# lhaippp/DMHomo

Hardware: AMD Instinct MI355X
Metric: sampled images/sec (128x128, s_step=32) (higher is better)
Workload: dtype f32; 1 GPU; DGM CFG-Unet dim=64 128x128 bs=25/GPU s_step=32 cond_scale=3 (BASELINE configs[1]); global_batch=25, cfg_mode=streams, hip_graph=True, weights=seeded random init

## Files before the change

dmhomo_amd/csrc/conv_f16x3.hip:

```cpp
#include <stdlib.h>

#include "common.h"

#include "conv_args.h"
#include "weight_image.h"

typedef _Float16 half8 __attribute__((ext_vector_type(8)));
typedef _Float16 half4 __attribute__((ext_vector_type(4)));
typedef float float4v __attribute__((ext_vector_type(4)));

namespace {

constexpr int KC = 32;
constexpr int PITCH = 160;
constexpr int STEP_U4 = 4 * 64;

template <int KH, int KW, int S, int UPS, int TH, int TW, int WM, int WN>
struct F16Cfg {
  static_assert(WM * WN == 4, "four waves per workgroup");
  static constexpr bool SUB = UPS == 3;
  static_assert(SUB || TH * TW == WM * 64, "64 pixels per wave");
  static_assert(!SUB || (KH == 2 && KW == 2 && S == 1 && TH == 4 && TW == 16 && WM == 4 && WN == 1), "sub-pixel geometry");
  static constexpr int IN_H = SUB ? TH + 2 : (TH - 1) * S + KH;
  static constexpr int IN_W = SUB ? TW + 2 : (TW - 1) * S + KW;
  static constexpr int IN_PIX = IN_H * IN_W;
  static constexpr int QS = UPS == 4 ? 2 : 3, NQ = 1 << QS;
  static constexpr int NLOAD = (IN_PIX * NQ + 255) / 256;
  static constexpr int PAD = UPS == 2 ? 0 : ((S == 1) ? (KH / 2) : (KH == 4 ? 1 : 0));
  static constexpr int ROWP = IN_W * PITCH;
  static constexpr int IN_BYTES = IN_H * ROWP;
  static constexpr int EPI_BYTES = 4 * 32 * EpilogueRows::EP * 4;
  static constexpr int TILE_BYTES = IN_BYTES > EPI_BYTES ? IN_BYTES : EPI_BYTES;
  static constexpr int LDS_BYTES = TILE_BYTES + 16;
};

__device__ __forceinline__ unsigned absbits(float x) { return __float_as_uint(x) & 0x7fffffffu; }

__device__ __forceinline__ int64_t f16x3_frag_floats_dev(int Cout, int C0, int C1, int T) {
  return (int64_t)((Cout + 63) / 64) * ((C0 + KC - 1) / KC + (C1 + KC - 1) / KC) * T * 2 * STEP_U4 * 4;
}

}

template <int KH, int KW, int S, int UPS, int TH, int TW, int WM, int WN>
__global__ __launch_bounds__(256, 2) void conv_f16x3_kernel(ConvArgs p) {
  using Cfg = F16Cfg<KH, KW, S, UPS, TH, TW, WM, WN>;
  constexpr bool PK = UPS == 4;
  constexpr int IN_W = Cfg::IN_W, IN_PIX = Cfg::IN_PIX, NLOAD = Cfg::NLOAD, NTAPS = PK ? (KH * KW + 1) / 2 : KH * KW,
                ROWP = Cfg::ROWP;

  extern __shared__ __attribute__((aligned(16))) float lds[];
  unsigned char* in_tile = reinterpret_cast<unsigned char*>(lds);
  unsigned* mxslot = reinterpret_cast<unsigned*>(in_tile + Cfg::TILE_BYTES);

  const int tid = threadIdx.x;
  const int lane = tid & 63;
  const int wave = tid >> 6;
  const int wave_u = __builtin_amdgcn_readfirstlane(wave);
  const int kg = lane >> 4;
  const int l15 = lane & 15;
  const int wm = wave / WN, wn = wave % WN;

  int t = blockIdx.x, by = blockIdx.y, nb = gridDim.x;
  if (p.rows) {
    nb = p.tilesX * p.tilesY * p.rows[0];
    const int lin = t + by * (int)gridDim.x;
    if (lin >= nb * (int)gridDim.y) return;
    t = lin % nb;
    by = lin / nb;
  }
  if (p.xcd) {
    const int total = nb * gridDim.y, lin = t + by * nb;
    const int q = total >> 3, r = total & 7, xcd = lin & 7, local = lin >> 3;
    const int nl = xcd * q + min(xcd, r) + local;
    if (p.xcd == 2) {
      by = nl % (int)gridDim.y;
      t = nl / (int)gridDim.y;
    } else {
      t = nl % nb;
      by = nl / nb;
    }
  }
  const int tx = t % p.tilesX;
  t /= p.tilesX;
  const int ty = t % p.tilesY;
  const int b = dmh_rows_phys(p.rows, t / p.tilesY);
  const int nt = UPS == 3 ? wm * (int)gridDim.y + by : by * WN + wn;
  const int n0 = UPS == 3 ? by * 64 : nt * 64;

  const int oy0 = ty * TH, ox0 = tx * TW;
  const int iy0 = oy0 * S - Cfg::PAD, ix0 = ox0 * S - Cfg::PAD;
  const int Hlim = UPS == 1 ? p.Hin * 2 : (UPS == 2 ? p.Hin / 2 + 1 : p.Hin);
  const int Wlim = UPS == 1 ? p.Win * 2 : (UPS == 2 ? p.Win / 2 + 1 : p.Win);

  if (tid < 2) mxslot[tid] = 0u;
#ifdef DMH_STAMPS
  unsigned long long tk[8] = {0, 0, 0, 0, 0, 0, 0, 0};
  unsigned long long t_prev, t_now;
#define STAMP(i)                                                                 \
  __builtin_amdgcn_sched_barrier(0);                                             \
  asm volatile("s_memtime %0\n\ts_waitcnt lgkmcnt(0)" : "=s"(t_now)::"memory"); \
  __builtin_amdgcn_sched_barrier(0);                                             \
  tk[i] += t_now - t_prev;                                                       \
  t_prev = t_now;
  asm volatile("s_memtime %0\n\ts_waitcnt lgkmcnt(0)" : "=s"(t_prev)::"memory");
  const unsigned long long t_begin = t_prev;
  const unsigned long long rt_begin = __builtin_amdgcn_s_memrealtime();
#else
#define STAMP(i)
#endif

  static_assert(TW == 16, "a 16-row MFMA block is one tile row");
  int arow[4];
#pragma unroll
  for (int mb = 0; mb < 4; ++mb)
    arow[mb] = UPS == 3 ? (mb + (wm >> 1)) * ROWP + (l15 + (wm & 1)) * PITCH + kg * 16
                        : ((wm * 4 + mb) * S) * ROWP + (l15 * S) * PITCH + (PK ? (kg & 1) : kg) * 16;

  float4v acc[4][4];
#pragma unroll
  for (int mb = 0; mb < 4; ++mb)
#pragma unroll
    for (int nb = 0; nb < 4; ++nb) acc[mb][nb] = float4v{0.f, 0.f, 0.f, 0.f};

  const int nchunks = p.nch0 + p.nch1;
  const int nsteps = nchunks * NTAPS * 2;
  const uint4* wbase = reinterpret_cast<const uint4*>(p.wpack) + (size_t)__builtin_amdgcn_readfirstlane(nt) * nsteps * STEP_U4;

  constexpr bool ROWREUSE = KH == 3 && KW == 3 && S == 1 && UPS != 3 && UPS != 2;
  constexpr int NSTEP = NTAPS * 2;
  constexpr int NB = (NSTEP % 3 == 0 && WN != 1) ? 3 : 2;
  uint4 bq[NB][4];
  auto tap_of = [](int pos) constexpr { return ROWREUSE ? (pos % 3) * 3 + pos / 3 : pos; };
  auto load_b = [&](int buf, int ch_, int st_) {
    if (st_ >= NSTEP) {
      st_ -= NSTEP;
      ch_ += 1;
    }
    if (ch_ >= nchunks) ch_ = nchunks - 1;
    const uint4* src = wbase + ((size_t)(ch_ * NTAPS + tap_of(st_ >> 1)) * 2 + (st_ & 1)) * STEP_U4;
#pragma unroll
    for (int i = 0; i < 4; ++i) bq[buf][i] = src[i * 64 + lane];
  };
#pragma unroll
  for (int i = 0; i < NB - 1; ++i) load_b(i, 0, i);

  constexpr int QS = Cfg::QS, NQ = Cfg::NQ;
  const int c4 = tid & (NQ - 1);
  float4 v[NLOAD];
  constexpr bool PACKPW = KH == 3 && KW == 3 && S == 1 && UPS == 0 && WN == 1;
  int poff[NLOAD], wroff[PACKPW ? 1 : NLOAD];
  const int y0c = min(max(iy0, 0), Hlim - 1), x0c = min(max(ix0, 0), Wlim - 1);
  const int pbase = PACKPW ? (b * p.Hin + y0c) * p.Win + x0c : 0;
  unsigned inside = 0;
#pragma unroll
  for (int i = 0; i < NLOAD; ++i) {
    const int pix = (tid + i * 256) >> QS;
    const int pixc = pix < IN_PIX ? pix : IN_PIX - 1;
    const int wro = (pixc / IN_W) * ROWP + (pixc % IN_W) * PITCH + c4 * 8;
    if (!PACKPW) wroff[i] = wro;
    const int yy = iy0 + pixc / IN_W, xx = ix0 + pixc % IN_W;
    const bool ok = pix < IN_PIX && yy >= 0 && yy < Hlim && xx >= 0 && xx < Wlim;
    const int yc = min(max(yy, 0), Hlim - 1), xc = min(max(xx, 0), Wlim - 1);
    const int sy = UPS == 1 ? (yc >> 1) : yc, sx = UPS == 1 ? (xc >> 1) : xc;
    poff[i] = UPS == 2 ? ((yc << 16) | xc) : (b * p.Hin + sy) * p.Win + sx;
    if (PACKPW) poff[i] = (int)((unsigned)wro | ((unsigned)((yc - y0c) * p.Win + (xc - x0c)) << 16));
    inside |= (ok ? 1u : 0u) << i;
  }
  unsigned inside_ch = inside;
  const float* ld_src = p.src0;
  int ld_C = p.C0, ld_c = 0, ld_py = 0, ld_px = 0;
  auto issue_prep = [&](int ch) {
    const bool s1 = ch >= p.nch0;
    ld_src = s1 ? p.src1 : p.src0;
    ld_C = s1 ? p.C1 : p.C0;
    if (UPS == 2) {
      const int nchc = p.C0 / KC, par = ch / nchc;
      ld_py = par >> 1;
      ld_px = par & 1;
      ld_c = (ch - par * nchc) * KC + c4 * 4;
      inside_ch = 0u;
    } else {
      const int c = (s1 ? ch - p.nch0 : ch) * KC + c4 * 4;
      ld_c = c < ld_C ? c : 0;
    }
  };
  auto issue_one = [&](int i) {
    const float* a;
    if (UPS == 2) {
      const int ry = 2 * (poff[i] >> 16) - 1 + ld_py, rx = 2 * (poff[i] & 0xffff) - 1 + ld_px;
      const bool ok = ((inside >> i) & 1u) && ry >= 0 && ry < p.Hin && rx >= 0 && rx < p.Win;
      const int yc = min(max(ry, 0), p.Hin - 1), xc = min(max(rx, 0), p.Win - 1);
      a = ld_src + ((size_t)(b * p.Hin + yc) * p.Win + xc) * ld_C + ld_c;
      inside_ch |= (ok ? 1u : 0u) << i;
    } else {
      if (PACKPW) a = ld_src + (size_t)pbase * ld_C + (int)(((unsigned)poff[i] >> 16) * (unsigned)ld_C + (unsigned)ld_c);
      else a = ld_src + (size_t)poff[i] * ld_C + ld_c;
    }
#ifdef DMH_STAMPS
    a = (p.ablate & 32) ? ld_src + ld_c : a;
#endif
    v[i] = ld4(a);
  };
  issue_prep(0);
#pragma unroll
  for (int i = 0; i < NLOAD; ++i) issue_one(i);
  __syncthreads();
#ifdef DMH_STAMPS
  if (p.ablate & 128) {
    const float* gs = p.src0 + (size_t)b * p.Hin * p.Win * p.C0;
    double q1 = 0.0, q2 = 0.0;
#pragma unroll
    for (int j = 0; j < 4; ++j) {
      const float2 t2 = *reinterpret_cast<const float2*>(gs + (size_t)(((tid & 31) + 32 * j) * 8 + (tid >> 5)) * 2);
      q1 += (double)t2.x;
      q2 += (double)t2.y;
    }
    for (int off = 16; off; off >>= 1) {
      q1 += __shfl_xor(q1, off);
      q2 += __shfl_xor(q2, off);
    }
    const double nn = (double)p.Hin * p.Win * (p.C0 / 8);
    const double mean = q1 / nn;
    double var = q2 / nn - mean * mean;
    var = var < 0.0 ? 0.0 : var;
    const float rstd = (float)(1.0 / sqrt(var + 1e-5)), meanf = (float)mean;
    float* tab = reinterpret_cast<float*>(in_tile);
    float* gtab = tab + 2 * 768;
    if ((tid & 31) == 0) {
      gtab[(tid >> 5) * 2 + 0] = meanf;
      gtab[(tid >> 5) * 2 + 1] = rstd;
    }
    __syncthreads();
    const float* cf = p.in_coef ? p.in_coef + (size_t)b * 2 * p.C0 : p.bias;
    for (int c = tid; c < p.C0 && c < 768; c += 256) {
      const int g8 = c / max(p.C0 / 8, 1);
      const float ga = cf ? cf[c % 64] : 1.f, be = cf ? cf[(c + 32) % 64] : 0.f;
      const float aa = gtab[g8 * 2 + 1] * ga;
      tab[c * 2 + 0] = aa;
      tab[c * 2 + 1] = be - gtab[g8 * 2 + 0] * aa;
    }
    __syncthreads();
    const float probe = tab[(tid & 63) * 2] + tab[(tid & 63) * 2 + 1];
    asm volatile("" ::"v"(probe));
    __syncthreads();
  }
#endif

  int e_run = 16;
  bool stat = p.in_bound != nullptr;
  int e_fix = 16;
  if (stat) {
    float m = 0.f;
    for (int i = 0; i < p.in_bound_n; ++i) {
      const float v = p.in_bound[b * p.in_bound_n + i];
      m = (v < INFINITY) ? fmaxf(m, v) : INFINITY;
    }
    const unsigned mb = __builtin_amdgcn_readfirstlane(__float_as_uint(m));
    stat = mb < 0x7f000000u;
    e_fix = min(max((int)(mb >> 23) + 1, 16), 254);
  }
  for (int ch = 0; ch < nchunks; ++ch) {
    const bool s1c = ch >= p.nch0;
    const bool pro = (p.in_coef != nullptr) && !s1c;
    float4 ca = make_float4(1.f, 1.f, 1.f, 1.f), cb = make_float4(0.f, 0.f, 0.f, 0.f);
    if (pro) {
      const int cq = ch * KC + c4 * 4;
      const int ccq = cq < p.C0 ? cq : 0;
      ca = ld4(p.in_coef + (size_t)(b * 2 + 0) * p.C0 + ccq);
      cb = ld4(p.in_coef + (size_t)(b * 2 + 1) * p.C0 + ccq);
    }
    const bool cvalid = UPS == 2 || (s1c ? ch - p.nch0 : ch) * KC + c4 * 4 < (s1c ? p.C1 : p.C0);
    const unsigned msk = cvalid ? inside_ch : 0u;
    if (pro) {
#pragma unroll
      for (int i = 0; i < NLOAD; ++i) {
        if ((i + 1) * 256 > IN_PIX * NQ && ((wave_u * 64 + i * 256) >> QS) >= IN_PIX) continue;
        v[i].x = silu_fast(fmaf(ca.x, v[i].x, cb.x));
        v[i].y = silu_fast(fmaf(ca.y, v[i].y, cb.y));
        v[i].z = silu_fast(fmaf(ca.z, v[i].z, cb.z));
        v[i].w = silu_fast(fmaf(ca.w, v[i].w, cb.w));
      }
    }
    if (!stat) {
      float mxf = 0.f;
#pragma unroll
      for (int i = 0; i < NLOAD; ++i) {
        if (pro && (i + 1) * 256 > IN_PIX * NQ && ((wave_u * 64 + i * 256) >> QS) >= IN_PIX) continue;
        mxf = fmaxf(fmaxf(mxf, fmaxf(fabsf(v[i].x), fabsf(v[i].y))), fmaxf(fabsf(v[i].z), fabsf(v[i].w)));
      }
      unsigned mx = __float_as_uint(mxf);
      mx = wave_max_u32(mx);
      if (lane == 0) atomicMax(&mxslot[ch & 1], mx);
    }
    STAMP(0)
    __syncthreads();
    STAMP(1)
    const int e_old = e_run;
    int e_ch = e_fix;
    if (!stat) {
      const unsigned bmx = mxslot[ch & 1];
      if (tid == 0) mxslot[(ch + 1) & 1] = 0u;
      e_ch = min(max((int)(__builtin_amdgcn_readfirstlane(bmx) >> 23), 16), 254);
    }
    e_run = max(e_run, e_ch);
    const float sc = __uint_as_float((unsigned)(268 - e_run) << 23);
    if (e_run != e_old && ch > 0) {
      const int fe = 127 + e_old - e_run;
      const float f = fe > 0 ? __uint_as_float((unsigned)fe << 23) : 0.f;
#pragma unroll
      for (int mb = 0; mb < 4; ++mb)
#pragma unroll
        for (int nb = 0; nb < 4; ++nb) acc[mb][nb] *= f;
    }
    const bool more = ch + 1 < nchunks;
    if (more) issue_prep(ch + 1);
#ifdef DMH_STAMPS
    if (p.ablate & 1) {
#pragma unroll
      for (int i = 0; i < NLOAD; ++i)
        if (more) issue_one(i);
    } else
#endif
#pragma unroll
    for (int i = 0; i < NLOAD; ++i) {
      if ((i + 1) * 256 <= IN_PIX * NQ || ((tid + i * 256) >> QS) < IN_PIX) {
        const float si = ((msk >> i) & 1u) ? sc : 0.f;
        uint2 h1, h2;
        dmh_split2(v[i].x, v[i].y, si, h1.x, h2.x);
        dmh_split2(v[i].z, v[i].w, si, h1.y, h2.y);
        int slot = PACKPW ? poff[i] : wroff[i];
        if (PACKPW) asm volatile("v_and_b32 %0, 0xffff, %0" : "+v"(slot));
        unsigned char* dst = in_tile + slot;
        *reinterpret_cast<uint2*>(dst) = h1;
        *reinterpret_cast<uint2*>(dst + 64) = h2;
      }
      if (more) issue_one(i);
    }
    STAMP(2)
    __syncthreads();
    STAMP(3)
    __builtin_amdgcn_sched_barrier(0);

    half8 a[4][2];
    half8 ar[ROWREUSE ? 5 : 1][2];
    auto read_a = [&](int tap) {
      const unsigned char* at = in_tile + (tap / KW) * ROWP + (tap % KW) * PITCH;
      if constexpr (PK) {
        const int t0 = 2 * tap, t1 = 2 * tap + 1 < KH * KW ? 2 * tap + 1 : 2 * tap;
        const int o0 = (t0 / KW) * ROWP + (t0 % KW) * PITCH, o1 = (t1 / KW) * ROWP + (t1 % KW) * PITCH;
        at = in_tile + ((kg >> 1) ? o1 : o0);
      }
#pragma unroll
      for (int mb = 0; mb < 4; ++mb)
#pragma unroll
        for (int pl = 0; pl < 2; ++pl) a[mb][pl] = *reinterpret_cast<const half8*>(at + arow[mb] + pl * 64);
    };
    auto read_rows = [&](int kx, int r0, int r1) {
      const unsigned char* at = in_tile + kx * PITCH;
#pragma unroll
      for (int r = r0; r < r1; ++r)
#pragma unroll
        for (int pl = 0; pl < 2; ++pl)
          ar[ROWREUSE ? r % 5 : 0][pl] = *reinterpret_cast<const half8*>(at + arow[0] + r * ROWP + pl * 64);
    };
#ifdef DMH_STAMPS
    if (!(p.ablate & 2))
#endif
    {
#pragma unroll
      for (int st = 0; st < NSTEP; ++st) {
#ifdef DMH_STAMPS
        if (!(p.ablate & 8))
#endif
        load_b((st + NB - 1) % NB, ch, st + NB - 1);
        __builtin_amdgcn_sched_barrier(0);
        const int pos = st >> 1;
#ifdef DMH_STAMPS
        if (!(p.ablate & 16) || st == 0)
#endif
        {
          if (ROWREUSE) {
            if ((st & 1) == 0) read_rows(pos / 3, pos % 3 == 0 ? 0 : 3 + pos % 3, 4 + pos % 3);
          } else if ((st & 1) == 0) {
            read_a(pos);
          }
        }
        auto afrag = [&](int mb, int pl) -> half8 {
          if constexpr (ROWREUSE) return ar[(mb + pos % 3) % 5][pl];
          else return a[mb][pl];
        };
#define DMH_A(mb, pl) afrag(mb, pl)
#pragma unroll
        for (int mb = 0; mb < 4; ++mb)
#pragma unroll
          for (int nb = 0; nb < 2; ++nb) {
            float4v& c = acc[mb][(st & 1) * 2 + nb];
            const half8 g1 = __builtin_bit_cast(half8, bq[st % NB][nb * 2]), g2 = __builtin_bit_cast(half8, bq[st % NB][nb * 2 + 1]);
            const half8 h1 = DMH_A(mb, 0), h2 = DMH_A(mb, 1);
            asm("v_mfma_f32_16x16x32_f16 %0, %1, %4, %0\n\t"
                "v_mfma_f32_16x16x32_f16 %0, %2, %3, %0\n\t"
                "v_mfma_f32_16x16x32_f16 %0, %1, %3, %0"
                : "+v"(c) : "v"(g1), "v"(g2), "v"(h1), "v"(h2));
          }
#undef DMH_A
      }
    }
#pragma unroll
    for (int mb = 0; mb < 4; mb += 2)
      asm volatile("s_nop 15" : "+v"(acc[mb][0]), "+v"(acc[mb][1]), "+v"(acc[mb][2]), "+v"(acc[mb][3]), "+v"(acc[mb + 1][0]),
                   "+v"(acc[mb + 1][1]), "+v"(acc[mb + 1][2]), "+v"(acc[mb + 1][3]));
    __builtin_amdgcn_sched_barrier(0);
    STAMP(4)
  }

#ifdef DMH_STAMPS
  if (!(p.ablate & 4))
#endif
  {
    constexpr int EP = EpilogueRows::EP;
    const float inv_s = __uint_as_float((unsigned)(e_run - 14) << 23);
    float* wl = lds + wave * (32 * EP);
    EpilogueRows er(p, b, n0);
    if (UPS == 3 && p.oscale) er.osc = ld4(p.oscale + nt * 64 + er.c4 * 4);
    er.osc.x *= inv_s;
    er.osc.y *= inv_s;
    er.osc.z *= inv_s;
    er.osc.w *= inv_s;
    __syncthreads();
#pragma unroll
    for (int hb = 0; hb < 2; ++hb) {
#pragma unroll
      for (int m2 = 0; m2 < 2; ++m2)
#pragma unroll
        for (int nb = 0; nb < 4; ++nb)
          *reinterpret_cast<float4v*>(wl + (m2 * 16 + l15) * EP + nb * 16 + kg * 4) = acc[hb * 2 + m2][nb];
      __builtin_amdgcn_fence(__ATOMIC_RELEASE, "wavefront");
      __builtin_amdgcn_wave_barrier();
      __builtin_amdgcn_fence(__ATOMIC_ACQUIRE, "wavefront");
      if (UPS == 3) er.template store_rows<TW>(p, wl, hb * 32, oy0, ox0, 2, wm >> 1, wm & 1);
      else er.template store_rows<TW, (KH == 1 && KW == 1 && WN == 1 && UPS == 0)>(p, wl, wm * 64 + hb * 32, oy0, ox0);
    }
#ifdef DMH_STAMPS
    STAMP(5)
    if (p.stats && lane == 0 && by == 0) {
      const int stiles = ((p.Hout + 7) / 8) * p.tilesX;
      unsigned long long* d = reinterpret_cast<unsigned long long*>(
                                  p.stats + ((size_t)(b * stiles + (ty * (TH / 8)) * p.tilesX + tx) * p.Cout) * 2) + wave * 8;
      for (int i = 0; i < 6; ++i) d[i] = tk[i];
      d[6] = t_now - t_begin;
      d[7] = __builtin_amdgcn_s_memrealtime() - rt_begin;
    }
#else
    er.template write_stats_grid<WM, WN, TH>(p, lds, ty, tx, by);
#endif
  }
}
#undef STAMP

__global__ __launch_bounds__(64) void f16x3_wscale_kernel(const float* __restrict__ w, float* __restrict__ oscale,
                                                           int Cout, int K) {
  const int o = blockIdx.x;
  float m = 0.f;
  if (o < Cout)
    for (int i = threadIdx.x; i < K; i += 64) m = fmaxf(m, fabsf(w[(size_t)o * K + i]));
  const float s = f16x3_row_scale(m);
  if (threadIdx.x == 0) oscale[o] = s;
}

__global__ void pack_f16x3_weight_kernel(const float* __restrict__ w, const float* __restrict__ oscale,
                                         _Float16* __restrict__ wp, int Cout, int C0, int NTAPS, int nch, int64_t total,
                                         int s2d) {
  const int64_t idx = (int64_t)blockIdx.x * blockDim.x + threadIdx.x;
  if (idx >= total) return;
  const F16x3Slot s = f16x3_slot(idx, NTAPS, nch);
  float ws = 0.f;
  if (s2d) {
    const int nchc = C0 / KC, par = s.ch / nchc;
    const int cr = (s.ch - par * nchc) * KC + s.k;
    const int ky = 2 * (s.tap >> 1) + (par >> 1), kx = 2 * (s.tap & 1) + (par & 1);
    if (s.o < Cout) ws = w[((size_t)s.o * C0 + cr) * 16 + ky * 4 + kx] / oscale[s.o];
  } else {
    const int tt = 2 * s.tap + (s.k >> 4), cc = s.k & 15;
    if (s.o < Cout && cc < C0 && tt < 49) ws = w[((size_t)s.o * C0 + cc) * 49 + tt] / oscale[s.o];
  }
  wp[idx] = f16x3_piece(ws, s.plane);
}

static int64_t f16x3_frag_floats(int Cout, int C0, int C1, int KH, int KW);
#define PM_MAX 32
struct PmTable {
  const float* src[PM_MAX];
  float* ws[PM_MAX];
  float* wpack[PM_MAX];
  int Cout[PM_MAX], C0[PM_MAX], C1[PM_MAX], T[PM_MAX], tr[PM_MAX];
  int blk0[PM_MAX + 1];
  int count;
};
__device__ __forceinline__ int pm_find(const PmTable& t, int blk) {
  int lo = 0, hi = t.count;
  while (hi - lo > 1) {
    const int mid = (lo + hi) >> 1;
    if (t.blk0[mid] <= blk) lo = mid; else hi = mid;
  }
  return lo;
}
__device__ __forceinline__ float pm_elem(const float* w, int o, int c, int tap, int Cout, int Cin, int T, int tr) {
  return tr ? w[((size_t)c * Cout + o) * T + (T - 1 - tap)] : w[((size_t)o * Cin + c) * T + tap];
}
__global__ __launch_bounds__(256) void pm_ws_kernel(PmTable t, float eps) {
  const int ti = pm_find(t, blockIdx.x), o = blockIdx.x - t.blk0[ti];
  const int K = (t.tr[ti] ? t.Cout[ti] : t.C0[ti] + t.C1[ti]) * t.T[ti];
  ws_standardize_row(t.src[ti] + (size_t)o * K, t.ws[ti] + (size_t)o * K, K, eps);
}
__global__ __launch_bounds__(64) void pm_wscale_kernel(PmTable t) {
  const int ti = pm_find(t, blockIdx.x), o = blockIdx.x - t.blk0[ti];
  const int Cout = t.Cout[ti], Cin = t.C0[ti] + t.C1[ti], T = t.T[ti], tr = t.tr[ti], K = Cin * T;
  const float* w = t.ws[ti] ? t.ws[ti] : t.src[ti];
  float m = 0.f;
  if (o < Cout)
    for (int i = threadIdx.x; i < K; i += 64) m = fmaxf(m, fabsf(pm_elem(w, o, i / T, i % T, Cout, Cin, T, tr)));
  const float sc = f16x3_row_scale(m);
  if (threadIdx.x == 0) t.wpack[ti][f16x3_frag_floats_dev(Cout, t.C0[ti], t.C1[ti], T) + o] = sc;
}
__global__ __launch_bounds__(256) void pm_pack_kernel(PmTable t) {
  const int ti = pm_find(t, blockIdx.x);
  const int Cout = t.Cout[ti], C0 = t.C0[ti], C1 = t.C1[ti], T = t.T[ti], tr = t.tr[ti];
  const int nch0 = (C0 + KC - 1) / KC, nch1 = (C1 + KC - 1) / KC;
  const int64_t frag = f16x3_frag_floats_dev(Cout, C0, C1, T);
  const int64_t total = frag * 2;
  const float* w = t.ws[ti] ? t.ws[ti] : t.src[ti];
  const float* oscale = t.wpack[ti] + frag;
  _Float16* wp = reinterpret_cast<_Float16*>(t.wpack[ti]);
  const int64_t base = (int64_t)(blockIdx.x - t.blk0[ti]) * 2048;
  for (int64_t idx = base + threadIdx.x; idx < min(base + 2048, total); idx += 256) {
    const F16x3Slot s = f16x3_slot(idx, T, nch0 + nch1);
    const bool src1 = s.ch >= nch0;
    const int c = (s.ch - (src1 ? nch0 : 0)) * KC + s.k;
    float ws = 0.f;
    if (c < (src1 ? C1 : C0) && s.o < Cout)
      ws = pm_elem(w, s.o, c + (src1 ? C0 : 0), s.tap, Cout, C0 + C1, T, tr) / oscale[s.o];
    wp[idx] = f16x3_piece(ws, s.plane);
  }
}

int dmh_f16x3_pack_multi(const DmhPackJob* jobs, int njobs, float eps, hipStream_t st) {
  for (int phase = 0; phase < 3; ++phase) {
    for (int i0 = 0; i0 < njobs;) {
      PmTable t;
      int k = 0, blocks = 0;
      for (; k < PM_MAX && i0 < njobs; ++i0) {
        const DmhPackJob& j = jobs[i0];
        if (phase == 0 && !j.ws) continue;
        const int T = j.KH * j.KH;
        t.src[k] = j.src;
        t.ws[k] = j.ws;
        t.wpack[k] = j.wpack;
        t.Cout[k] = j.Cout;
        t.C0[k] = j.C0;
        t.C1[k] = j.C1;
        t.T[k] = T;
        t.tr[k] = j.transposed;
        t.blk0[k] = blocks;
        if (phase == 0) blocks += j.transposed ? j.C0 + j.C1 : j.Cout;
        else if (phase == 1) blocks += cdiv(j.Cout, 64) * 64;
        else blocks += (int)cdiv64(f16x3_frag_floats(j.Cout, j.C0, j.C1, j.KH, j.KH) * 2, 2048);
        ++k;
      }
      if (k == 0) continue;
      t.blk0[k] = blocks;
      t.count = k;
      if (phase == 0) hipLaunchKernelGGL(pm_ws_kernel, dim3(blocks), dim3(256), 0, st, t, eps);
      else if (phase == 1) hipLaunchKernelGGL(pm_wscale_kernel, dim3(blocks), dim3(64), 0, st, t);
      else hipLaunchKernelGGL(pm_pack_kernel, dim3(blocks), dim3(256), 0, st, t);
      DMH_CHECK_LAUNCH("dmh_pack_conv_weights_multi");
    }
  }
  return DMH_OK;
}

static bool f16x3_pk(int C0, int C1, int KH) { return KH == 7 && C1 == 0 && C0 <= 16; }

static int64_t f16x3_frag_floats(int Cout, int C0, int C1, int KH, int KW) {
  if (KH == 4) return (int64_t)cdiv(Cout, 64) * (4 * C0 / KC) * 4 * 2 * STEP_U4 * 4;
  if (f16x3_pk(C0, C1, KH)) return (int64_t)cdiv(Cout, 64) * 25 * 2 * STEP_U4 * 4;
  return (int64_t)cdiv(Cout, 64) * (cdiv(C0, KC) + cdiv(C1, KC)) * KH * KW * 2 * STEP_U4 * 4;
}

int64_t dmh_f16x3_pack_floats(int Cout, int C0, int C1, int KH, int KW) {
  return f16x3_frag_floats(Cout, C0, C1, KH, KW) + (int64_t)cdiv(Cout, 64) * 64;
}

int dmh_f16x3_pack(const float* w, float* wpack, int Cout, int C0, int C1, int KH, int KW, hipStream_t st) {
  const bool s2d = KH == 4;
  if (!s2d && !f16x3_pk(C0, C1, KH)) {
    const DmhPackJob job = {w, nullptr, wpack, Cout, C0, C1, KH, 0};
    return dmh_f16x3_pack_multi(&job, 1, 0.f, st);
  }
  const int64_t frag = f16x3_frag_floats(Cout, C0, C1, KH, KW);
  float* oscale = wpack + frag;
  hipLaunchKernelGGL(f16x3_wscale_kernel, dim3(cdiv(Cout, 64) * 64), dim3(64), 0, st, w, oscale, Cout, C0 * KH * KW);
  const int64_t total = frag * 2;
  hipLaunchKernelGGL(pack_f16x3_weight_kernel, dim3((unsigned)cdiv64(total, 256)), dim3(256), 0, st, w, oscale,
                     reinterpret_cast<_Float16*>(wpack), Cout, C0, s2d ? 4 : 25, s2d ? 4 * C0 / KC : 1, total, s2d ? 1 : 0);
  DMH_CHECK_LAUNCH("dmh_pack_conv_weight(f16x3)");
  return DMH_OK;
}

template <int KH, int KW, int S, int UPS, int TH, int TW, int WM, int WN>
static int launch_f16x3(const DmhConv* d, int Hout, int Wout, hipStream_t st) {
  using Cfg = F16Cfg<KH, KW, S, UPS, TH, TW, WM, WN>;
  ConvArgs a = fill_conv_args(d, Hout, Wout, KC, TH, TW);
  if (UPS == 2) a.nch0 = 4 * a.C0 / KC;
  a.oscale = d->wpack + f16x3_frag_floats(d->Cout, a.C0, a.C1, UPS == 2 ? 4 : KH, UPS == 2 ? 4 : KW);
#ifdef DMH_STAMPS
  if (const char* e = getenv("DMH_WINO_ABLATE")) a.ablate = atoi(e);
#endif
  auto kern = conv_f16x3_kernel<KH, KW, S, UPS, TH, TW, WM, WN>;
  DMH_RAISE_LDS_ONCE(kern, Cfg::LDS_BYTES, "dmh_conv2d(f16x3)");
  static const int xcd_deep = [] {
    const char* e = getenv("DMH_CONV_XCD_DEEP");
    return e ? atoi(e) : 32;
  }();
  if (xcd_deep > 0 && Hout <= xcd_deep && cdiv(a.Cout, 64 * WN) > 1) a.xcd = 2;
  dim3 grid(a.tilesX * a.tilesY * a.B, cdiv(a.Cout, 64 * WN));
  hipLaunchKernelGGL(kern, grid, dim3(256), Cfg::LDS_BYTES, st, a);
  DMH_CHECK_LAUNCH("dmh_conv2d(f16x3)");
  return DMH_OK;
}

__global__ void subpixel_weight_kernel(const float* __restrict__ w, float* __restrict__ wv, int Cout, int Cin) {
  const int64_t idx = (int64_t)blockIdx.x * blockDim.x + threadIdx.x;
  const int64_t total = (int64_t)4 * Cout * Cin * 4;
  if (idx >= total) return;
  const int tb = idx & 1, ta = (idx >> 1) & 1;
  int64_t r = idx >> 2;
  const int c = r % Cin;
  r /= Cin;
  const int o = r % Cout, par = r / Cout;
  const int dy = par >> 1, dx = par & 1;
  const int ky0 = dy == 0 ? (ta == 0 ? 0 : 1) : (ta == 0 ? 0 : 2), ky1 = dy == 0 ? (ta == 0 ? 0 : 2) : (ta == 0 ? 1 : 2);
  const int kx0 = dx == 0 ? (tb == 0 ? 0 : 1) : (tb == 0 ? 0 : 2), kx1 = dx == 0 ? (tb == 0 ? 0 : 2) : (tb == 0 ? 1 : 2);
  const float* wk = w + ((size_t)o * Cin + c) * 9;
  float s = 0.f;
  for (int ky = ky0; ky <= ky1; ++ky)
    for (int kx = kx0; kx <= kx1; ++kx) s += wk[ky * 3 + kx];
  wv[idx] = s;
}

int64_t dmh_f16x3_up2_pack_floats(int Cout, int C0) {
  return dmh_f16x3_pack_floats(4 * Cout, C0, 0, 2, 2) + (int64_t)16 * Cout * C0;
}

int dmh_f16x3_up2_pack(const float* w, float* wpack, int Cout, int C0, hipStream_t st) {
  float* wv = wpack + dmh_f16x3_pack_floats(4 * Cout, C0, 0, 2, 2);
  const int64_t total = (int64_t)16 * Cout * C0;
  hipLaunchKernelGGL(subpixel_weight_kernel, dim3((unsigned)cdiv64(total, 256)), dim3(256), 0, st, w, wv, Cout, C0);
  return dmh_f16x3_pack(wv, wpack, 4 * Cout, C0, 0, 2, 2, st);
}

int dmh_f16x3_launch_up2(const DmhConv* d, int Hout, int Wout, hipStream_t st) {
  using Cfg = F16Cfg<2, 2, 1, 3, 4, 16, 4, 1>;
  ConvArgs a = fill_conv_args(d, Hout, Wout, KC, 4, 16);
  a.tilesX = cdiv(d->Win, 16);
  a.tilesY = cdiv(d->Hin, 4);
  a.oscale = d->wpack + f16x3_frag_floats(4 * d->Cout, a.C0, 0, 2, 2);
  auto kern = conv_f16x3_kernel<2, 2, 1, 3, 4, 16, 4, 1>;
  DMH_RAISE_LDS_ONCE(kern, Cfg::LDS_BYTES, "dmh_conv2d(f16x3 sub-pixel)");
  dim3 grid(a.tilesX * a.tilesY * a.B, cdiv(a.Cout, 64));
  hipLaunchKernelGGL(kern, grid, dim3(256), Cfg::LDS_BYTES, st, a);
  DMH_CHECK_LAUNCH("dmh_conv2d(f16x3 sub-pixel)");
  return DMH_OK;
}

int dmh_f16x3_launch(const DmhConv* d, int Hout, int Wout, hipStream_t st) {
  const bool wide = d->Cout % 128 == 0;
  if (d->KH == 4) {
    return wide ? launch_f16x3<2, 2, 1, 2, 8, 16, 2, 2>(d, Hout, Wout, st)
                : launch_f16x3<2, 2, 1, 2, 16, 16, 4, 1>(d, Hout, Wout, st);
  }
  if (d->KH == 7) {
    if (f16x3_pk(d->C0, d->src1 ? d->C1 : 0, 7)) return launch_f16x3<7, 7, 1, 4, 16, 16, 4, 1>(d, Hout, Wout, st);
    return launch_f16x3<7, 7, 1, 0, 16, 16, 4, 1>(d, Hout, Wout, st);
  }
  if (d->KH == 1) {
    return wide ? launch_f16x3<1, 1, 1, 0, 8, 16, 2, 2>(d, Hout, Wout, st)
                : launch_f16x3<1, 1, 1, 0, 16, 16, 4, 1>(d, Hout, Wout, st);
  }
  if (d->upsample2) {
    return wide ? launch_f16x3<3, 3, 1, 1, 8, 16, 2, 2>(d, Hout, Wout, st)
                : launch_f16x3<3, 3, 1, 1, 16, 16, 4, 1>(d, Hout, Wout, st);
  }
  if (wide) return launch_f16x3<3, 3, 1, 0, 8, 16, 2, 2>(d, Hout, Wout, st);
  DMH_REQUIRE(17 * (int64_t)d->Win + 17 < 65536, "dmh_conv2d: 3x3 with Cout %% 128 != 0 supports Win <= 3853 (got %d)", d->Win);
  return launch_f16x3<3, 3, 1, 0, 16, 16, 4, 1>(d, Hout, Wout, st);
}
```

Before: 89.70 images/s.

## Split K across two wave groups for small-spatial 3x3 convolutions

Adds a KS=2 variant of the f16x3 conv kernel in which a 512-thread workgroup splits the input-channel chunks between two halves. Each half keeps its own LDS tile and exponent scale, and the partial accumulators are reduced through LDS before the epilogue. It is used for 3x3 convs with at most 256 output pixels, Cout at most 256 and at least 8 K chunks. The aim is more parallelism and latency hiding in the deep low-resolution U-Net layers, where the grid is small. In exchange it uses more LDS, allows only one block per CU, and adds a reduction step with extra barriers.

After: 89.92 images/s, median of 4. No clear change (+0.2%).

```diff
diff --git a/dmhomo_amd/csrc/conv_f16x3.hip b/dmhomo_amd/csrc/conv_f16x3.hip
--- a/dmhomo_amd/csrc/conv_f16x3.hip
+++ b/dmhomo_amd/csrc/conv_f16x3.hip
@@ -14,10 +14,12 @@
 constexpr int KC = 32;
 constexpr int PITCH = 160;
 constexpr int STEP_U4 = 4 * 64;
-
-template <int KH, int KW, int S, int UPS, int TH, int TW, int WM, int WN>
+constexpr int cmax(int a, int b) { return a > b ? a : b; }
+
+template <int KH, int KW, int S, int UPS, int TH, int TW, int WM, int WN, int KS = 1>
 struct F16Cfg {
-  static_assert(WM * WN == 4, "four waves per workgroup");
+  static_assert(WM * WN == 4, "four waves per workgroup (per K half)");
+  static_assert(KS == 1 || (KS == 2 && WM == 2 && WN == 2 && UPS == 0 && S == 1), "K split: two halves of the 2x2 layout");
   static constexpr bool SUB = UPS == 3;
   static_assert(SUB || TH * TW == WM * 64, "64 pixels per wave");
   static_assert(!SUB || (KH == 2 && KW == 2 && S == 1 && TH == 4 && TW == 16 && WM == 4 && WN == 1), "sub-pixel geometry");
@@ -30,7 +32,8 @@
   static constexpr int ROWP = IN_W * PITCH;
   static constexpr int IN_BYTES = IN_H * ROWP;
   static constexpr int EPI_BYTES = 4 * 32 * EpilogueRows::EP * 4;
-  static constexpr int TILE_BYTES = IN_BYTES > EPI_BYTES ? IN_BYTES : EPI_BYTES;
+  static constexpr int RED_BYTES = KS == 2 ? 4 * 64 * 64 * 4 : 0;
+  static constexpr int TILE_BYTES = cmax(cmax(KS * IN_BYTES, EPI_BYTES), RED_BYTES);
   static constexpr int LDS_BYTES = TILE_BYTES + 16;
 };
 
@@ -42,18 +45,20 @@
 
 }
 
-template <int KH, int KW, int S, int UPS, int TH, int TW, int WM, int WN>
-__global__ __launch_bounds__(256, 2) void conv_f16x3_kernel(ConvArgs p) {
-  using Cfg = F16Cfg<KH, KW, S, UPS, TH, TW, WM, WN>;
+template <int KH, int KW, int S, int UPS, int TH, int TW, int WM, int WN, int KS = 1>
+__global__ __launch_bounds__(256 * KS, KS == 1 ? 2 : 1) void conv_f16x3_kernel(ConvArgs p) {
+  using Cfg = F16Cfg<KH, KW, S, UPS, TH, TW, WM, WN, KS>;
   constexpr bool PK = UPS == 4;
   constexpr int IN_W = Cfg::IN_W, IN_PIX = Cfg::IN_PIX, NLOAD = Cfg::NLOAD, NTAPS = PK ? (KH * KW + 1) / 2 : KH * KW,
                 ROWP = Cfg::ROWP;
 
+  const int half = KS == 1 ? 0 : __builtin_amdgcn_readfirstlane((int)threadIdx.x >> 8);
+
   extern __shared__ __attribute__((aligned(16))) float lds[];
-  unsigned char* in_tile = reinterpret_cast<unsigned char*>(lds);
-  unsigned* mxslot = reinterpret_cast<unsigned*>(in_tile + Cfg::TILE_BYTES);
-
-  const int tid = threadIdx.x;
+  unsigned char* in_tile = reinterpret_cast<unsigned char*>(lds) + half * Cfg::IN_BYTES;
+  unsigned* mxslot = reinterpret_cast<unsigned*>(reinterpret_cast<unsigned char*>(lds) + Cfg::TILE_BYTES) + half * 2;
+
+  const int tid = KS == 1 ? threadIdx.x : (threadIdx.x & 255);
   const int lane = tid & 63;
   const int wave = tid >> 6;
   const int wave_u = __builtin_amdgcn_readfirstlane(wave);
@@ -125,7 +130,8 @@
 
   const int nchunks = p.nch0 + p.nch1;
   const int nsteps = nchunks * NTAPS * 2;
-  const uint4* wbase = reinterpret_cast<const uint4*>(p.wpack) + (size_t)__builtin_amdgcn_readfirstlane(nt) * nsteps * STEP_U4;
+  const int wt = KS == 1 ? nt : min(nt, (p.Cout + 63) / 64 - 1);
+  const uint4* wbase = reinterpret_cast<const uint4*>(p.wpack) + (size_t)__builtin_amdgcn_readfirstlane(wt) * nsteps * STEP_U4;
 
   constexpr bool ROWREUSE = KH == 3 && KW == 3 && S == 1 && UPS != 3 && UPS != 2;
   constexpr int NSTEP = NTAPS * 2;
@@ -135,7 +141,7 @@
   auto load_b = [&](int buf, int ch_, int st_) {
     if (st_ >= NSTEP) {
       st_ -= NSTEP;
-      ch_ += 1;
+      ch_ += KS;
     }
     if (ch_ >= nchunks) ch_ = nchunks - 1;
     const uint4* src = wbase + ((size_t)(ch_ * NTAPS + tap_of(st_ >> 1)) * 2 + (st_ & 1)) * STEP_U4;
@@ -143,7 +149,7 @@
     for (int i = 0; i < 4; ++i) bq[buf][i] = src[i * 64 + lane];
   };
 #pragma unroll
-  for (int i = 0; i < NB - 1; ++i) load_b(i, 0, i);
+  for (int i = 0; i < NB - 1; ++i) load_b(i, half, i);
 
   constexpr int QS = Cfg::QS, NQ = Cfg::NQ;
   const int c4 = tid & (NQ - 1);
@@ -202,7 +208,7 @@
 #endif
     v[i] = ld4(a);
   };
-  issue_prep(0);
+  issue_prep(KS == 1 ? 0 : min(half, nchunks - 1));
 #pragma unroll
   for (int i = 0; i < NLOAD; ++i) issue_one(i);
   __syncthreads();
@@ -260,7 +266,8 @@
     stat = mb < 0x7f000000u;
     e_fix = min(max((int)(mb >> 23) + 1, 16), 254);
   }
-  for (int ch = 0; ch < nchunks; ++ch) {
+  for (int ch = half; ch - half < nchunks; ch += KS) {
+    const bool active = KS == 1 || ch < nchunks;
     const bool s1c = ch >= p.nch0;
     const bool pro = (p.in_coef != nullptr) && !s1c;
     float4 ca = make_float4(1.f, 1.f, 1.f, 1.f), cb = make_float4(0.f, 0.f, 0.f, 0.f);
@@ -282,7 +289,7 @@
         v[i].w = silu_fast(fmaf(ca.w, v[i].w, cb.w));
       }
     }
-    if (!stat) {
+    if (!stat && active) {
       float mxf = 0.f;
 #pragma unroll
       for (int i = 0; i < NLOAD; ++i) {
@@ -291,126 +298,129 @@
       }
       unsigned mx = __float_as_uint(mxf);
       mx = wave_max_u32(mx);
-      if (lane == 0) atomicMax(&mxslot[ch & 1], mx);
+      if (lane == 0) atomicMax(&mxslot[(ch / KS) & 1], mx);
     }
     STAMP(0)
     __syncthreads();
     STAMP(1)
-    const int e_old = e_run;
-    int e_ch = e_fix;
-    if (!stat) {
-      const unsigned bmx = mxslot[ch & 1];
-      if (tid == 0) mxslot[(ch + 1) & 1] = 0u;
-      e_ch = min(max((int)(__builtin_amdgcn_readfirstlane(bmx) >> 23), 16), 254);
-    }
-    e_run = max(e_run, e_ch);
-    const float sc = __uint_as_float((unsigned)(268 - e_run) << 23);
-    if (e_run != e_old && ch > 0) {
-      const int fe = 127 + e_old - e_run;
-      const float f = fe > 0 ? __uint_as_float((unsigned)fe << 23) : 0.f;
-#pragma unroll
-      for (int mb = 0; mb < 4; ++mb)
-#pragma unroll
-        for (int nb = 0; nb < 4; ++nb) acc[mb][nb] *= f;
-    }
-    const bool more = ch + 1 < nchunks;
-    if (more) issue_prep(ch + 1);
-#ifdef DMH_STAMPS
-    if (p.ablate & 1) {
-#pragma unroll
-      for (int i = 0; i < NLOAD; ++i)
+    if (active) {
+      const int e_old = e_run;
+      int e_ch = e_fix;
+      if (!stat) {
+        const unsigned bmx = mxslot[(ch / KS) & 1];
+        if (tid == 0) mxslot[(ch / KS + 1) & 1] = 0u;
+        e_ch = min(max((int)(__builtin_amdgcn_readfirstlane(bmx) >> 23), 16), 254);
+      }
+      e_run = max(e_run, e_ch);
+      const float sc = __uint_as_float((unsigned)(268 - e_run) << 23);
+      if (e_run != e_old && ch >= KS) {
+        const int fe = 127 + e_old - e_run;
+        const float f = fe > 0 ? __uint_as_float((unsigned)fe << 23) : 0.f;
+#pragma unroll
+        for (int mb = 0; mb < 4; ++mb)
+#pragma unroll
+          for (int nb = 0; nb < 4; ++nb) acc[mb][nb] *= f;
+      }
+      const bool more = ch + KS < nchunks;
+      if (more) issue_prep(ch + KS);
+#ifdef DMH_STAMPS
+      if (p.ablate & 1) {
+#pragma unroll
+        for (int i = 0; i < NLOAD; ++i)
+          if (more) issue_one(i);
+      } else
+#endif
+#pragma unroll
+      for (int i = 0; i < NLOAD; ++i) {
+        if ((i + 1) * 256 <= IN_PIX * NQ || ((tid + i * 256) >> QS) < IN_PIX) {
+          const float si = ((msk >> i) & 1u) ? sc : 0.f;
+          uint2 h1, h2;
+          dmh_split2(v[i].x, v[i].y, si, h1.x, h2.x);
+          dmh_split2(v[i].z, v[i].w, si, h1.y, h2.y);
+          int slot = PACKPW ? poff[i] : wroff[i];
+          if (PACKPW) asm volatile("v_and_b32 %0, 0xffff, %0" : "+v"(slot));
+          unsigned char* dst = in_tile + slot;
+          *reinterpret_cast<uint2*>(dst) = h1;
+          *reinterpret_cast<uint2*>(dst + 64) = h2;
+        }
         if (more) issue_one(i);
-    } else
-#endif
-#pragma unroll
-    for (int i = 0; i < NLOAD; ++i) {
-      if ((i + 1) * 256 <= IN_PIX * NQ || ((tid + i * 256) >> QS) < IN_PIX) {
-        const float si = ((msk >> i) & 1u) ? sc : 0.f;
-        uint2 h1, h2;
-        dmh_split2(v[i].x, v[i].y, si, h1.x, h2.x);
-        dmh_split2(v[i].z, v[i].w, si, h1.y, h2.y);
-        int slot = PACKPW ? poff[i] : wroff[i];
-        if (PACKPW) asm volatile("v_and_b32 %0, 0xffff, %0" : "+v"(slot));
-        unsigned char* dst = in_tile + slot;
-        *reinterpret_cast<uint2*>(dst) = h1;
-        *reinterpret_cast<uint2*>(dst + 64) = h2;
-      }
-      if (more) issue_one(i);
+      }
     }
     STAMP(2)
     __syncthreads();
     STAMP(3)
     __builtin_amdgcn_sched_barrier(0);
-
-    half8 a[4][2];
-    half8 ar[ROWREUSE ? 5 : 1][2];
-    auto read_a = [&](int tap) {
-      const unsigned char* at = in_tile + (tap / KW) * ROWP + (tap % KW) * PITCH;
-      if constexpr (PK) {
-        const int t0 = 2 * tap, t1 = 2 * tap + 1 < KH * KW ? 2 * tap + 1 : 2 * tap;
-        const int o0 = (t0 / KW) * ROWP + (t0 % KW) * PITCH, o1 = (t1 / KW) * ROWP + (t1 % KW) * PITCH;
-        at = in_tile + ((kg >> 1) ? o1 : o0);
-      }
-#pragma unroll
-      for (int mb = 0; mb < 4; ++mb)
-#pragma unroll
-        for (int pl = 0; pl < 2; ++pl) a[mb][pl] = *reinterpret_cast<const half8*>(at + arow[mb] + pl * 64);
-    };
-    auto read_rows = [&](int kx, int r0, int r1) {
-      const unsigned char* at = in_tile + kx * PITCH;
-#pragma unroll
-      for (int r = r0; r < r1; ++r)
-#pragma unroll
-        for (int pl = 0; pl < 2; ++pl)
-          ar[ROWREUSE ? r % 5 : 0][pl] = *reinterpret_cast<const half8*>(at + arow[0] + r * ROWP + pl * 64);
-    };
-#ifdef DMH_STAMPS
-    if (!(p.ablate & 2))
-#endif
-    {
-#pragma unroll
-      for (int st = 0; st < NSTEP; ++st) {
-#ifdef DMH_STAMPS
-        if (!(p.ablate & 8))
-#endif
-        load_b((st + NB - 1) % NB, ch, st + NB - 1);
-        __builtin_amdgcn_sched_barrier(0);
-        const int pos = st >> 1;
-#ifdef DMH_STAMPS
-        if (!(p.ablate & 16) || st == 0)
-#endif
-        {
-          if (ROWREUSE) {
-            if ((st & 1) == 0) read_rows(pos / 3, pos % 3 == 0 ? 0 : 3 + pos % 3, 4 + pos % 3);
-          } else if ((st & 1) == 0) {
-            read_a(pos);
+    if (active) {
+      half8 a[4][2];
+      half8 ar[ROWREUSE ? 5 : 1][2];
+      auto read_a = [&](int tap) {
+        const unsigned char* at = in_tile + (tap / KW) * ROWP + (tap % KW) * PITCH;
+        if constexpr (PK) {
+          const int t0 = 2 * tap, t1 = 2 * tap + 1 < KH * KW ? 2 * tap + 1 : 2 * tap;
+          const int o0 = (t0 / KW) * ROWP + (t0 % KW) * PITCH, o1 = (t1 / KW) * ROWP + (t1 % KW) * PITCH;
+          at = in_tile + ((kg >> 1) ? o1 : o0);
+        }
+#pragma unroll
+        for (int mb = 0; mb < 4; ++mb)
+#pragma unroll
+          for (int pl = 0; pl < 2; ++pl) a[mb][pl] = *reinterpret_cast<const half8*>(at + arow[mb] + pl * 64);
+      };
+      auto read_rows = [&](int kx, int r0, int r1) {
+        const unsigned char* at = in_tile + kx * PITCH;
+#pragma unroll
+        for (int r = r0; r < r1; ++r)
+#pragma unroll
+          for (int pl = 0; pl < 2; ++pl)
+            ar[ROWREUSE ? r % 5 : 0][pl] = *reinterpret_cast<const half8*>(at + arow[0] + r * ROWP + pl * 64);
+      };
+#ifdef DMH_STAMPS
+      if (!(p.ablate & 2))
+#endif
+      {
+#pragma unroll
+        for (int st = 0; st < NSTEP; ++st) {
+#ifdef DMH_STAMPS
+          if (!(p.ablate & 8))
+#endif
+          load_b((st + NB - 1) % NB, ch, st + NB - 1);
+          __builtin_amdgcn_sched_barrier(0);
+          const int pos = st >> 1;
+#ifdef DMH_STAMPS
+          if (!(p.ablate & 16) || st == 0)
+#endif
+          {
+            if (ROWREUSE) {
+              if ((st & 1) == 0) read_rows(pos / 3, pos % 3 == 0 ? 0 : 3 + pos % 3, 4 + pos % 3);
+            } else if ((st & 1) == 0) {
+              read_a(pos);
+            }
           }
+          auto afrag = [&](int mb, int pl) -> half8 {
+            if constexpr (ROWREUSE) return ar[(mb + pos % 3) % 5][pl];
+            else return a[mb][pl];
+          };
+#define DMH_A(mb, pl) afrag(mb, pl)
+#pragma unroll
+          for (int mb = 0; mb < 4; ++mb)
+#pragma unroll
+            for (int nb = 0; nb < 2; ++nb) {
+              float4v& c = acc[mb][(st & 1) * 2 + nb];
+              const half8 g1 = __builtin_bit_cast(half8, bq[st % NB][nb * 2]), g2 = __builtin_bit_cast(half8, bq[st % NB][nb * 2 + 1]);
+              const half8 h1 = DMH_A(mb, 0), h2 = DMH_A(mb, 1);
+              asm("v_mfma_f32_16x16x32_f16 %0, %1, %4, %0\n\t"
+                  "v_mfma_f32_16x16x32_f16 %0, %2, %3, %0\n\t"
+                  "v_mfma_f32_16x16x32_f16 %0, %1, %3, %0"
+                  : "+v"(c) : "v"(g1), "v"(g2), "v"(h1), "v"(h2));
+            }
+#undef DMH_A
         }
-        auto afrag = [&](int mb, int pl) -> half8 {
-          if constexpr (ROWREUSE) return ar[(mb + pos % 3) % 5][pl];
-          else return a[mb][pl];
-        };
-#define DMH_A(mb, pl) afrag(mb, pl)
-#pragma unroll
-        for (int mb = 0; mb < 4; ++mb)
-#pragma unroll
-          for (int nb = 0; nb < 2; ++nb) {
-            float4v& c = acc[mb][(st & 1) * 2 + nb];
-            const half8 g1 = __builtin_bit_cast(half8, bq[st % NB][nb * 2]), g2 = __builtin_bit_cast(half8, bq[st % NB][nb * 2 + 1]);
-            const half8 h1 = DMH_A(mb, 0), h2 = DMH_A(mb, 1);
-            asm("v_mfma_f32_16x16x32_f16 %0, %1, %4, %0\n\t"
-                "v_mfma_f32_16x16x32_f16 %0, %2, %3, %0\n\t"
-                "v_mfma_f32_16x16x32_f16 %0, %1, %3, %0"
-                : "+v"(c) : "v"(g1), "v"(g2), "v"(h1), "v"(h2));
-          }
-#undef DMH_A
-      }
-    }
-#pragma unroll
-    for (int mb = 0; mb < 4; mb += 2)
-      asm volatile("s_nop 15" : "+v"(acc[mb][0]), "+v"(acc[mb][1]), "+v"(acc[mb][2]), "+v"(acc[mb][3]), "+v"(acc[mb + 1][0]),
-                   "+v"(acc[mb + 1][1]), "+v"(acc[mb + 1][2]), "+v"(acc[mb + 1][3]));
-    __builtin_amdgcn_sched_barrier(0);
+      }
+#pragma unroll
+      for (int mb = 0; mb < 4; mb += 2)
+        asm volatile("s_nop 15" : "+v"(acc[mb][0]), "+v"(acc[mb][1]), "+v"(acc[mb][2]), "+v"(acc[mb][3]), "+v"(acc[mb + 1][0]),
+                     "+v"(acc[mb + 1][1]), "+v"(acc[mb + 1][2]), "+v"(acc[mb + 1][3]));
+      __builtin_amdgcn_sched_barrier(0);
+    }
     STAMP(4)
   }
 
@@ -419,31 +429,57 @@
 #endif
   {
     constexpr int EP = EpilogueRows::EP;
+    if constexpr (KS == 2) {
+      float4v* red = reinterpret_cast<float4v*>(lds) + wave * (16 * 64) + lane;
+      __syncthreads();
+      if (half) {
+#pragma unroll
+        for (int mb = 0; mb < 4; ++mb)
+#pragma unroll
+          for (int nb = 0; nb < 4; ++nb) red[(mb * 4 + nb) * 64] = acc[mb][nb];
+        if (tid == 0) mxslot[0] = (unsigned)e_run;
+      }
+      __syncthreads();
+      if (!half) {
+        const int e_oth = __builtin_amdgcn_readfirstlane((int)mxslot[2]);
+        const int e_fin = max(e_run, e_oth);
+        const int fo = 127 + e_run - e_fin, ft = 127 + e_oth - e_fin;
+        const float f_own = fo > 0 ? __uint_as_float((unsigned)fo << 23) : 0.f;
+        const float f_oth = ft > 0 ? __uint_as_float((unsigned)ft << 23) : 0.f;
+#pragma unroll
+        for (int mb = 0; mb < 4; ++mb)
+#pragma unroll
+          for (int nb = 0; nb < 4; ++nb) acc[mb][nb] = acc[mb][nb] * f_own + red[(mb * 4 + nb) * 64] * f_oth;
+        e_run = e_fin;
+      }
+    }
     const float inv_s = __uint_as_float((unsigned)(e_run - 14) << 23);
-    float* wl = lds + wave * (32 * EP);
+    float* wl = lds + wave * (KS == 2 ? 16 * 64 * 4 : 32 * EP);
     EpilogueRows er(p, b, n0);
     if (UPS == 3 && p.oscale) er.osc = ld4(p.oscale + nt * 64 + er.c4 * 4);
     er.osc.x *= inv_s;
     er.osc.y *= inv_s;
     er.osc.z *= inv_s;
     er.osc.w *= inv_s;
-    __syncthreads();
-#pragma unroll
-    for (int hb = 0; hb < 2; ++hb) {
-#pragma unroll
-      for (int m2 = 0; m2 < 2; ++m2)
-#pragma unroll
-        for (int nb = 0; nb < 4; ++nb)
-          *reinterpret_cast<float4v*>(wl + (m2 * 16 + l15) * EP + nb * 16 + kg * 4) = acc[hb * 2 + m2][nb];
-      __builtin_amdgcn_fence(__ATOMIC_RELEASE, "wavefront");
-      __builtin_amdgcn_wave_barrier();
-      __builtin_amdgcn_fence(__ATOMIC_ACQUIRE, "wavefront");
-      if (UPS == 3) er.template store_rows<TW>(p, wl, hb * 32, oy0, ox0, 2, wm >> 1, wm & 1);
-      else er.template store_rows<TW, (KH == 1 && KW == 1 && WN == 1 && UPS == 0)>(p, wl, wm * 64 + hb * 32, oy0, ox0);
+    if (KS == 1) __syncthreads();
+    if (KS == 1 || !half) {
+#pragma unroll
+      for (int hb = 0; hb < 2; ++hb) {
+#pragma unroll
+        for (int m2 = 0; m2 < 2; ++m2)
+#pragma unroll
+          for (int nb = 0; nb < 4; ++nb)
+            *reinterpret_cast<float4v*>(wl + (m2 * 16 + l15) * EP + nb * 16 + kg * 4) = acc[hb * 2 + m2][nb];
+        __builtin_amdgcn_fence(__ATOMIC_RELEASE, "wavefront");
+        __builtin_amdgcn_wave_barrier();
+        __builtin_amdgcn_fence(__ATOMIC_ACQUIRE, "wavefront");
+        if (UPS == 3) er.template store_rows<TW>(p, wl, hb * 32, oy0, ox0, 2, wm >> 1, wm & 1);
+        else er.template store_rows<TW, (KH == 1 && KW == 1 && WN == 1 && UPS == 0)>(p, wl, wm * 64 + hb * 32, oy0, ox0);
+      }
     }
 #ifdef DMH_STAMPS
     STAMP(5)
-    if (p.stats && lane == 0 && by == 0) {
+    if (p.stats && lane == 0 && by == 0 && !half) {
       const int stiles = ((p.Hout + 7) / 8) * p.tilesX;
       unsigned long long* d = reinterpret_cast<unsigned long long*>(
                                   p.stats + ((size_t)(b * stiles + (ty * (TH / 8)) * p.tilesX + tx) * p.Cout) * 2) + wave * 8;
@@ -607,16 +643,16 @@
   return DMH_OK;
 }
 
-template <int KH, int KW, int S, int UPS, int TH, int TW, int WM, int WN>
+template <int KH, int KW, int S, int UPS, int TH, int TW, int WM, int WN, int KS = 1>
 static int launch_f16x3(const DmhConv* d, int Hout, int Wout, hipStream_t st) {
-  using Cfg = F16Cfg<KH, KW, S, UPS, TH, TW, WM, WN>;
+  using Cfg = F16Cfg<KH, KW, S, UPS, TH, TW, WM, WN, KS>;
   ConvArgs a = fill_conv_args(d, Hout, Wout, KC, TH, TW);
   if (UPS == 2) a.nch0 = 4 * a.C0 / KC;
   a.oscale = d->wpack + f16x3_frag_floats(d->Cout, a.C0, a.C1, UPS == 2 ? 4 : KH, UPS == 2 ? 4 : KW);
 #ifdef DMH_STAMPS
   if (const char* e = getenv("DMH_WINO_ABLATE")) a.ablate = atoi(e);
 #endif
-  auto kern = conv_f16x3_kernel<KH, KW, S, UPS, TH, TW, WM, WN>;
+  auto kern = conv_f16x3_kernel<KH, KW, S, UPS, TH, TW, WM, WN, KS>;
   DMH_RAISE_LDS_ONCE(kern, Cfg::LDS_BYTES, "dmh_conv2d(f16x3)");
   static const int xcd_deep = [] {
     const char* e = getenv("DMH_CONV_XCD_DEEP");
@@ -624,7 +660,7 @@
   }();
   if (xcd_deep > 0 && Hout <= xcd_deep && cdiv(a.Cout, 64 * WN) > 1) a.xcd = 2;
   dim3 grid(a.tilesX * a.tilesY * a.B, cdiv(a.Cout, 64 * WN));
-  hipLaunchKernelGGL(kern, grid, dim3(256), Cfg::LDS_BYTES, st, a);
+  hipLaunchKernelGGL(kern, grid, dim3(256 * KS), Cfg::LDS_BYTES, st, a);
   DMH_CHECK_LAUNCH("dmh_conv2d(f16x3)");
   return DMH_OK;
 }
@@ -691,6 +727,8 @@
     return wide ? launch_f16x3<3, 3, 1, 1, 8, 16, 2, 2>(d, Hout, Wout, st)
                 : launch_f16x3<3, 3, 1, 1, 16, 16, 4, 1>(d, Hout, Wout, st);
   }
+  if (Hout * Wout <= 256 && d->Cout <= 256 && cdiv(d->C0, KC) + (d->src1 ? cdiv(d->C1, KC) : 0) >= 8)
+    return launch_f16x3<3, 3, 1, 0, 8, 16, 2, 2, 2>(d, Hout, Wout, st);
   if (wide) return launch_f16x3<3, 3, 1, 0, 8, 16, 2, 2>(d, Hout, Wout, st);
   DMH_REQUIRE(17 * (int64_t)d->Win + 17 < 65536, "dmh_conv2d: 3x3 with Cout %% 128 != 0 supports Win <= 3853 (got %d)", d->Win);
   return launch_f16x3<3, 3, 1, 0, 16, 16, 4, 1>(d, Hout, Wout, st);
```
